# viridityzhu/HiFiHR

Hardware: AMD Instinct MI355X
Metric: train images/sec, FreiHAND 224x224 (ResNet-18 + MANO LBS + render + losses + Adam) (higher is better)
Workload: dtype f32; 1 GPU; BASELINE configs[1]: FreiHAND batch=32/GPU, ResNet-18 encoder + MANO LBS + silhouette/texture render losses, 224x224, aa=3 (672^2 samples); per_gpu_batch=32, global_batch=32, parallelism=dp1

## Files before the change

### hifihr_amd/csrc/conv_halo.hip

```cpp
#include <hip/hip_runtime.h>

#include <cstdlib>
#include <type_traits>

#include "hifihr_internal.h"
#include "lds_dma.h"

namespace hifihr {

namespace {

constexpr int kTW = 14, kTH = 8;
constexpr int kHP = 16;
constexpr int kHaloPix = (kTH + 2) * kHP;
constexpr int kPixF = 68;
constexpr int kHaloPieces = (kHaloPix * kPixF * 4 + 1023) / 1024;
constexpr int kHalo = (kHaloPieces + 1) / 2 * 2 * 256;
constexpr int kWStage = 64 * 64;
constexpr int kStages = 4;
constexpr int kTaps = 9;
constexpr int kNL = 4;
constexpr int kHaloPer = (kHaloPieces + kNL - 1) / kNL;
static_assert(2 * (kTaps - 3) >= kHaloPer, "the next tile's halo is issued two pieces per tap and must land two taps before the tile ends");

// ... 475 lines not shown
      for (int c = 0; c < 4; ++c) R[c] = addsub(raw[c], raw[4 + c], kBneg[i]);
#pragma unroll
      for (int j = 0; j < 4; ++j) {
        V[j] = addsub(R[kBa[j]], R[kBb[j]], kBneg[j]);
        if (HIFIHR_W2_ABLATE == 4) V[j] = raw[j];
      }
    };
    auto fold = [&](int i) {
#pragma unroll
      for (int j = 0; j < 4; ++j)
#pragma unroll
        for (int p = 0; p < 4; ++p) {
          const int co = kAt[p >> 1][i] * kAt[p & 1][j];
          if (co == 1) {
#pragma unroll
            for (int c = 0; c < NCB; ++c) Y[p][c] += M[j][c];
          } else if (co == -1) {
#pragma unroll
            for (int c = 0; c < NCB; ++c) Y[p][c] -= M[j][c];
          }
        }
    };
    read_raw(0);
#if defined(HIFIHR_HALO_STAMP)
    const unsigned long long l0 = HALO_T(), r0 = __builtin_amdgcn_s_memrealtime();
#endif
#pragma unroll
    for (int s = 0; s < kW2Stages; ++s, ++gs) {
#pragma unroll
      for (int q = 0; q < 2; ++q) {
        const int Q = 2 * s + q;
        if (q == 0) {
          read_w(gs, 0, 0);
          if ((s & 1) == 0 && s > 0) fold((s >> 1) - 1);
        }
        transform(Q);
        if (Q + 1 < 2 * kW2Stages) read_raw(Q + 1);
#pragma unroll
        for (int j = 0; j < 4; ++j) {
          if (j < 3) read_w(gs, q, j + 1);
          else if (q == 0) read_w(gs, 1, 0);
#pragma unroll
          for (int k = 0; k < 4; ++k)
#pragma unroll
            for (int c = 0; c < NCB; ++c) {
              const floatx4 acc = ((Q & 3) == 0 && k == 0) ? floatx4{0.f, 0.f, 0.f, 0.f} : M[j][c];
              M[j][c] = __builtin_amdgcn_mfma_f32_16x16x4f32(reinterpret_cast<const float*>(&wv[j & 1][c])[k], comp(V[j], k), acc, 0, 0, 0);
            }
          HIFIHR_SCHED_GROUP(0x100, NCB);
          HIFIHR_SCHED_GROUP(0x008, 4 * NCB);
          HIFIHR_PIN();
        }
      }
#if defined(HIFIHR_HALO_STAMP)
      HIFIHR_TOUCH(M[0][0][0]);
      const unsigned long long b0 = HALO_T();
#endif
      HIFIHR_RAW_BARRIER();
#if defined(HIFIHR_HALO_STAMP)
      st_bar += HALO_T() - b0;
#endif
    }
#if defined(HIFIHR_HALO_STAMP)
    const unsigned long long l1 = HALO_T();
    st_loop += l1 - l0; st_real += __builtin_amdgcn_s_memrealtime() - r0;
#endif
    fold(3);
    if (tt < (t.rows >> 1) * 7 && t.x0 + 2 * (tt % 7) < a.W) {
      const int ty2 = tt / 7, tx2 = tt - 7 * ty2;
#pragma unroll
      for (int c = 0; c < NCB; ++c) {
        const int ch = 16 * (cb0 + c) + 4 * g;
        float4 b4 = make_float4(0.f, 0.f, 0.f, 0.f);
        float4 r4[4] = {b4, b4, b4, b4};
        if constexpr (EPI) {
          if (a.bias != nullptr) b4 = *reinterpret_cast<const float4*>(a.bias + ch);
          if (a.res != nullptr) {
#pragma unroll
            for (int p = 0; p < 4; ++p)
              r4[p] = *reinterpret_cast<const float4*>(a.res + (((size_t)t.n * a.H + t.y0 + 2 * ty2 + (p >> 1)) * a.W + t.x0 + 2 * tx2 + (p & 1)) * 64 + ch);
          }
        }
        auto put = [&](float (&k4)[4], float (&s4)[4], float (&q4)[4], int& n) {
#pragma unroll
          for (int p = 0; p < 4; ++p) {
            float* o = a.dst + (((size_t)t.n * a.H + t.y0 + 2 * ty2 + (p >> 1)) * a.W + t.x0 + 2 * tx2 + (p & 1)) * 64 + ch;
            float4 v = make_float4(Y[p][c][0], Y[p][c][1], Y[p][c][2], Y[p][c][3]);
            if constexpr (EPI) {
              v.x += b4.x + r4[p].x; v.y += b4.y + r4[p].y; v.z += b4.z + r4[p].z; v.w += b4.w + r4[p].w;
              if (a.relu) { v.x = fmaxf(v.x, 0.f); v.y = fmaxf(v.y, 0.f); v.z = fmaxf(v.z, 0.f); v.w = fmaxf(v.w, 0.f); }
            }
            *reinterpret_cast<float4*>(o) = v;
            if constexpr (STATS) {
#if HIFIHR_W2_ABLATE != 7
            if (n == 0) { k4[0] = v.x; k4[1] = v.y; k4[2] = v.z; k4[3] = v.w; }
            const float d0 = v.x - k4[0], d1 = v.y - k4[1], d2 = v.z - k4[2], d3 = v.w - k4[3];
            s4[0] += d0; q4[0] += d0 * d0; s4[1] += d1; q4[1] += d1 * d1;
            s4[2] += d2; q4[2] += d2 * d2; s4[3] += d3; q4[3] += d3 * d3;
            ++n;
#endif
            }
          }
        };
        if (NCB == 2 ? c == 0 : rbw == 0) put(sk[0], ssum[0], ssq[0], sn[0]);
        else put(sk[1], ssum[1], ssq[1], sn[1]);
      }
    }
#if defined(HIFIHR_HALO_STAMP)
    st_epi += HALO_T() - l1;
#endif
  };
  for (int ti = 0; ti < ntiles; ++ti) {
    const Tile t = tile_of(a.H, a.ctiles, cur, s_hi, s_lo, lead);
    cur += t.rows;
    if (t.rows > 4) run_tile(std::integral_constant<int, 2>{}, t, ti & 1);
    else run_tile(std::integral_constant<int, 1>{}, t, ti & 1);
  }
#if defined(HIFIHR_HALO_STAMP)
  if (tid == 0) {
    atomicAdd(&g_halo_stamp[0], st_loop); atomicAdd(&g_halo_stamp[1], st_real); atomicAdd(&g_halo_stamp[2], (unsigned long long)nst);
    atomicAdd(&g_halo_stamp[3], st_bar); atomicAdd(&g_halo_stamp[4], 1ull); atomicAdd(&g_halo_stamp[5], HALO_T() - st_entry);
    atomicAdd(&g_halo_stamp[6], st_epi);
  }
#endif
  if (STATS && a.stats != nullptr) {
#pragma unroll
    for (int s = 0; s < 2; ++s) {
      double S1[4], S2[4];
#pragma unroll
      for (int e = 0; e < 4; ++e) {
        stat_unshift(sn[s], sk[s][e], ssum[s][e], ssq[s][e], S1[e], S2[e]);
        for (int o = 1; o < 16; o <<= 1) { S1[e] += __shfl_xor(S1[e], o, 64); S2[e] += __shfl_xor(S2[e], o, 64); }
      }
      if (r == 0) {
        double* sp = reinterpret_cast<double*>(a.stats) + (size_t)(wg & (stat_slots_used(64) - 1)) * 2 * 64 + 32 * chw + 16 * s + 4 * g;
#pragma unroll
        for (int e = 0; e < 4; ++e) { stat_atomic_add(sp + e, S1[e]); stat_atomic_add(sp + 64 + e, S2[e]); }
      }
    }
  }
}

template <bool EPI, bool STATS>
__global__ __launch_bounds__(256 + 64 * kNL) void conv_wino2_kernel(Wino2Args a) {
  __shared__ __attribute__((aligned(1024))) float lds[2 * kHalo + 2 * kW2Stage];
  wino2_body<EPI, STATS>(a, lds, (int)blockIdx.x, (int)gridDim.x);
}

namespace {
constexpr int kDyT = kTH * kTW * 64;
constexpr int kWgBuf = kHalo + kDyT;
constexpr int kWgPieces = kHaloPieces + kTH * kTW / 4;
constexpr int kWgPer = (kWgPieces + kNL - 1) / kNL;
struct HaloWgradArgs {
  const float* x;
  const float* dy;
  float* slabs;
  const float* zeros;
  int N, H, W;
  int ctiles, total, per;
};
}

__device__ __forceinline__ void halo_wgrad_body(const HaloWgradArgs& a, float* __restrict__ lds, int bid, int nblk) {
  const int tid = threadIdx.x, lane = tid & 63, wave = tid >> 6;
  const int wg = xcd_remap(bid, nblk);
  HaloArgs sh;
  sh.H = a.H; sh.ctiles = a.ctiles;
  const int s_lo = wg * a.per, s_hi = min(s_lo + a.per, a.total);
  int ntiles = 0;
  for (int cur = s_lo; cur < s_hi; cur += tile_at(sh, cur, s_hi).rows) ++ntiles;

  if (wave >= 4) {
    const int l = wave - 4;
    HIFIHR_SET_LOADER_PRIO();
    int pk[kWgPer];
#pragma unroll
    for (int i = 0; i < kWgPer; ++i) {
      const int q = l + kNL * i;
      if (q < kHaloPieces) {
        const int o = q * 1024 + lane * 16;
        const int hp = o / (kPixF * 4), within = o - hp * (kPixF * 4);
        pk[i] = (hp < kHaloPix && within < 256) ? ((hp >> 4) << 12) | ((hp & 15) << 8) | (within >> 4) : -1;
      } else {
        const int p = 4 * (q - kHaloPieces) + (lane >> 4), ty = p / kTW;
        pk[i] = (ty << 16) | ((p - ty * kTW) << 8) | (lane & 15);
      }
    }
    auto issue_tile = [&](const Tile& t, int buf) {
      float* base = lds + buf * kWgBuf;
      const float* ximg = a.x + (size_t)t.n * a.H * a.W * 64;
      const float* dyt = a.dy + (((size_t)t.n * a.H + t.y0) * a.W + t.x0) * 64;
#pragma unroll
      for (int i = 0; i < kWgPer; ++i) {
        const int q = l + kNL * i;
        if (q < kHaloPieces) {
          const int iy = t.y0 - 1 + (pk[i] >> 12), ix = t.x0 - 1 + ((pk[i] >> 8) & 15);
          const bool ok = pk[i] >= 0 && iy >= 0 && iy < a.H && ix >= 0 && ix < a.W;
          HIFIHR_GLDS16(ok ? ximg + (iy * a.W + ix) * 64 + (pk[i] & 15) * 4 : a.zeros, base + 256 * q, lane);
        } else if (q < kWgPieces) {
          const int ty = pk[i] >> 16, tx = (pk[i] >> 8) & 255;
          HIFIHR_GLDS16(ty < t.rows ? dyt + (ty * a.W + tx) * 64 + (pk[i] & 255) * 4 : a.zeros, base + kHalo + 256 * (q - kHaloPieces), lane);
        }
      }
    };
    int cur = s_lo;
    Tile t = tile_at(sh, cur, s_hi);
    if (ntiles > 0) issue_tile(t, 0);
    HIFIHR_WAIT_VM(0);
    HIFIHR_RAW_BARRIER();
    for (int ti = 0; ti < ntiles; ++ti) {
      cur += t.rows;
      if (ti + 1 < ntiles) {
        t = tile_at(sh, cur, s_hi);
        issue_tile(t, (ti + 1) & 1);
      }
      HIFIHR_WAIT_VM(0);
      HIFIHR_RAW_BARRIER();
    }
    return;
  }

  const int r = lane & 15, g = lane >> 4;
  floatx4 acc[kTaps][4];
#pragma unroll
  for (int tp = 0; tp < kTaps; ++tp)
#pragma unroll
    for (int m = 0; m < 4; ++m) acc[tp][m] = floatx4{0.f, 0.f, 0.f, 0.f};
  const char* const lds_b = reinterpret_cast<const char*>(lds);
  const int dy_lane = kHalo * 4 + (4 * r + wave) * 4;
  const int hx_lane = r * 16;

  HIFIHR_RAW_BARRIER();
  int cur = s_lo;
  for (int ti = 0; ti < ntiles; ++ti) {
    const Tile t = tile_at(sh, cur, s_hi);
    cur += t.rows;
    const char* const buf = lds_b + (ti & 1) * (kWgBuf * 4);
    const int ngroups = (t.rows * kTW + 3) >> 2;
    float fy[2];
    float4 fx[2][kTaps];
    auto read_group = [&](int P, int slot) {
      P = min(P, kTH * kTW / 4 - 1);
      const int tpix = 4 * P + g, ty = tpix / kTW;
      const int hpix = ty * kHP + (tpix - ty * kTW);
      fy[slot] = *reinterpret_cast<const float*>(buf + dy_lane + tpix * 256);
      const char* hb = buf + hx_lane + hpix * (kPixF * 4);
#pragma unroll
      for (int tp = 0; tp < kTaps; ++tp) fx[slot][tp] = *reinterpret_cast<const float4*>(hb + ((tp / 3) * kHP + (tp % 3)) * (kPixF * 4));
    };
    auto mfma_group = [&](int slot) {
#pragma unroll
      for (int tp = 0; tp < kTaps; ++tp) {
        acc[tp][0] = __builtin_amdgcn_mfma_f32_16x16x4f32(fy[slot], fx[slot][tp].x, acc[tp][0], 0, 0, 0);
        acc[tp][1] = __builtin_amdgcn_mfma_f32_16x16x4f32(fy[slot], fx[slot][tp].y, acc[tp][1], 0, 0, 0);
        acc[tp][2] = __builtin_amdgcn_mfma_f32_16x16x4f32(fy[slot], fx[slot][tp].z, acc[tp][2], 0, 0, 0);
        acc[tp][3] = __builtin_amdgcn_mfma_f32_16x16x4f32(fy[slot], fx[slot][tp].w, acc[tp][3], 0, 0, 0);
      }
    };
    auto interleave = [&]() {
#pragma unroll
      for (int i = 0; i < kTaps + 1; ++i) {
        HIFIHR_SCHED_GROUP(0x008, 3);
        HIFIHR_SCHED_GROUP(0x100, 1);
        HIFIHR_SCHED_GROUP(0x002, 2);
      }
      HIFIHR_SCHED_GROUP(0x008, 4 * kTaps - 3 * (kTaps + 1));
    };
    read_group(0, 0);
    for (int P = 0; P < ngroups; P += 2) {
      read_group(P + 1, 1);
      mfma_group(0);
      interleave();
      HIFIHR_PIN();
      read_group(P + 2, 0);
      if (P + 1 < ngroups) mfma_group(1);
      interleave();
      HIFIHR_PIN();
    }
    HIFIHR_RAW_BARRIER();
  }
  float* slab = a.slabs + (size_t)wg * (kTaps * 64 * 64);
#pragma unroll
  for (int tp = 0; tp < kTaps; ++tp)
#pragma unroll
    for (int e = 0; e < 4; ++e) {
      const int k = 4 * (4 * g + e) + wave;
      *reinterpret_cast<float4*>(slab + ((size_t)tp * 64 + k) * 64 + 4 * r) = make_float4(acc[tp][0][e], acc[tp][1][e], acc[tp][2][e], acc[tp][3][e]);
    }
}

__global__ __launch_bounds__(256 + 64 * kNL) void conv_halo_wgrad_kernel(HaloWgradArgs a) {
  __shared__ __attribute__((aligned(1024))) float lds[2 * kWgBuf];
  halo_wgrad_body(a, lds, (int)blockIdx.x, (int)gridDim.x);
}

template <bool EPI>
__global__ __launch_bounds__(256 + 64 * kNL) void conv_c64_bwd_pair_kernel(Wino2Args d, int ga, HaloWgradArgs w) {
  constexpr int kPairLds = 2 * kHalo + 2 * kW2Stage > 2 * kWgBuf ? 2 * kHalo + 2 * kW2Stage : 2 * kWgBuf;
  __shared__ __attribute__((aligned(1024))) float lds[kPairLds];
  const int b = (int)blockIdx.x;
  if (b < ga) wino2_body<EPI, false>(d, lds, b, ga);
  else halo_wgrad_body(w, lds, b - ga, (int)gridDim.x - ga);
}

__device__ __forceinline__ void halo_wgrad_reduce_body(const float* __restrict__ slabs, int nslab, float* __restrict__ dw, int blk) {
  __shared__ float part[4][64];
  const int lane = threadIdx.x & 63, w = threadIdx.x >> 6;
  const int i = blk * 64 + lane;
  constexpr size_t kSlab = (size_t)kTaps * 64 * 64;
  float s = 0.f;
  for (int z0 = 16 * w; z0 < nslab; z0 += 64) {
    float v[16];
#pragma unroll
    for (int u = 0; u < 16; ++u) v[u] = (z0 + u < nslab) ? slabs[(size_t)(z0 + u) * kSlab + i] : 0.f;
#pragma unroll
    for (int u = 0; u < 16; ++u) s += v[u];
  }
  part[w][lane] = s;
  __syncthreads();
  if (w == 0) {
    const int c = i & 63, k = (i >> 6) & 63, tp = i >> 12;
    dw[((size_t)k * kTaps + tp) * 64 + c] += (part[0][lane] + part[1][lane]) + (part[2][lane] + part[3][lane]);
  }
}
__global__ __launch_bounds__(256) void conv_halo_wgrad_reduce_kernel(const float* __restrict__ slabs, int nslab, float* __restrict__ dw) {
  halo_wgrad_reduce_body(slabs, nslab, dw, (int)blockIdx.x);
}
constexpr int kHaloReduceMaxJobs = 16;
struct HaloReduceJobs {
  const float* slabs[kHaloReduceMaxJobs];
  float* dw[kHaloReduceMaxJobs];
  int nslab[kHaloReduceMaxJobs];
};
__global__ __launch_bounds__(256) void conv_halo_wgrad_reduce_multi_kernel(HaloReduceJobs js) {
  const int j = blockIdx.y;
  halo_wgrad_reduce_body(js.slabs[j], js.nslab[j], js.dw[j], (int)blockIdx.x);
}

namespace {
constexpr int kSWP = 228;
constexpr int kSHP = 36;
constexpr int kSHRows = 2 * kTH + 5;
constexpr int kSHalo = kSHRows * kSHP * 4;
constexpr int kSPieces = (kSHalo * 4 + 1023) / 1024;
constexpr int kSHaloAl = kSPieces * 256;
struct StemArgs {
  const float* src;
  const float* wgt;
  float* dst;
  float* stats;
  const float* zeros;
  int N, IH, IW, OH, OW;
  int ctiles, total, per;
};
}

__global__ __launch_bounds__(384) void conv_stem_kernel(StemArgs a) {
  __shared__ __attribute__((aligned(1024))) float lds[64 * kSWP + 2 * kSHaloAl];
  float* const wl = lds;
  float* const halo = lds + 64 * kSWP;
  const int tid = threadIdx.x, lane = tid & 63, wave = tid >> 6;
  const int wg = xcd_remap((int)blockIdx.x, (int)gridDim.x);
  HaloArgs sh;
  sh.H = a.OH; sh.ctiles = a.ctiles;
  const int s_lo = wg * a.per, s_hi = min(s_lo + a.per, a.total);
  int ntiles = 0;
  for (int cur = s_lo; cur < s_hi; cur += tile_at(sh, cur, s_hi).rows) ++ntiles;
  __shared__ int c3_any;
  if (tid == 0) c3_any = 0;
  __syncthreads();
  bool c3_mine = false;
  for (int e = tid; e < 64 * 7 * 8; e += 384) {
    const int n = e / 56, rem = e - n * 56, tr = rem >> 3, sl = rem & 7;
    float4 v = make_float4(0.f, 0.f, 0.f, 0.f);
    if (sl < 7) v = *reinterpret_cast<const float4*>(a.wgt + ((size_t)(n * 7 + tr) * 7 + sl) * 4);
    c3_mine = c3_mine || v.w != 0.f;
    *reinterpret_cast<float4*>(wl + n * kSWP + (tr * 8 + sl) * 4) = v;
  }
  if (c3_mine) c3_any = 1;

  if (wave >= 4) {
    HIFIHR_SET_LOADER_PRIO();
    const int l = wave - 4;
    int pk[kSPieces / 2];
#pragma unroll
    for (int i = 0; i < kSPieces / 2; ++i) {
      const int hp = 64 * (l + 2 * i) + lane, hy = hp / kSHP, hx = hp - hy * kSHP;
      pk[i] = (hy < kSHRows && hx < 2 * kTW + 5) ? (hy << 8) | hx : -1;
    }
    auto issue_tile = [&](const Tile& t, int buf) {
      const float* ximg = a.src + (size_t)t.n * a.IH * a.IW * 4;
#pragma unroll
      for (int i = 0; i < kSPieces / 2; ++i) {
        const int iy = 2 * t.y0 - 3 + (pk[i] >> 8), ix = 2 * t.x0 - 3 + (pk[i] & 255);
        const bool ok = pk[i] >= 0 && iy >= 0 && iy < a.IH && ix >= 0 && ix < a.IW;
        HIFIHR_GLDS16(ok ? ximg + (iy * a.IW + ix) * 4 : a.zeros, halo + buf * kSHaloAl + 256 * (l + 2 * i), lane);
      }
    };
    int cur = s_lo;
    Tile t = tile_at(sh, cur, s_hi);
    if (ntiles > 0) issue_tile(t, 0);
    HIFIHR_WAIT_VM(0);
    __syncthreads();
    for (int ti = 0; ti < ntiles; ++ti) {
      cur += t.rows;
      if (ti + 1 < ntiles) {
        t = tile_at(sh, cur, s_hi);
        issue_tile(t, (ti + 1) & 1);
      }
      HIFIHR_WAIT_VM(0);
      HIFIHR_RAW_BARRIER();
    }
    return;
  }

  const int r = lane & 15, g = lane >> 4;
  int hoff[7];
#pragma unroll
  for (int j = 0; j < 7; ++j) {
    const int p = 16 * j + r, ty = p / kTW;
    hoff[j] = ((2 * ty) * kSHP + 2 * (p - ty * kTW) + g) * 16;
  }
  const int woff = (16 * wave + r) * (kSWP * 4) + g * 16;
  const char* const wl_b = reinterpret_cast<const char*>(wl);
  const char* const halo_b = reinterpret_cast<const char*>(halo);
  float ssum[4] = {0.f, 0.f, 0.f, 0.f}, ssq[4] = {0.f, 0.f, 0.f, 0.f}, sk[4] = {0.f, 0.f, 0.f, 0.f};
  int sn = 0;
  __syncthreads();
  const bool c3 = c3_any != 0;
  int cur = s_lo;
  for (int ti = 0; ti < ntiles; ++ti) {
    const Tile t = tile_at(sh, cur, s_hi);
    cur += t.rows;
    const char* const hb = halo_b + (ti & 1) * (kSHaloAl * 4);
    floatx4 acc[7];
#pragma unroll
    for (int j = 0; j < 7; ++j) acc[j] = floatx4{0.f, 0.f, 0.f, 0.f};
    float4 fw[2], fx[2][7];
    auto read_step = [&](int st, int slot) {
      const int tr = st >> 1, kk = st & 1;
      fw[slot] = *reinterpret_cast<const float4*>(wl_b + woff + (tr * 8 + 4 * kk) * 16);
      const char* hs = hb + (tr * kSHP + 4 * kk) * 16;
#pragma unroll
      for (int j = 0; j < 7; ++j) fx[slot][j] = *reinterpret_cast<const float4*>(hs + hoff[j]);
    };
    auto mfma_step = [&](int slot) {
#pragma unroll
      for (int j = 0; j < 7; ++j) acc[j] = __builtin_amdgcn_mfma_f32_16x16x4f32(fw[slot].x, fx[slot][j].x, acc[j], 0, 0, 0);
#pragma unroll
      for (int j = 0; j < 7; ++j) acc[j] = __builtin_amdgcn_mfma_f32_16x16x4f32(fw[slot].y, fx[slot][j].y, acc[j], 0, 0, 0);
#pragma unroll
      for (int j = 0; j < 7; ++j) acc[j] = __builtin_amdgcn_mfma_f32_16x16x4f32(fw[slot].z, fx[slot][j].z, acc[j], 0, 0, 0);
      if (c3) {
#pragma unroll
        for (int j = 0; j < 7; ++j) acc[j] = __builtin_amdgcn_mfma_f32_16x16x4f32(fw[slot].w, fx[slot][j].w, acc[j], 0, 0, 0);
      }
    };
    auto interleave = [&]() {
#pragma unroll
      for (int i = 0; i < 8; ++i) {
        HIFIHR_SCHED_GROUP(0x008, 2);
        HIFIHR_SCHED_GROUP(0x100, 1);
        HIFIHR_SCHED_GROUP(0x002, 1);
      }
      HIFIHR_SCHED_GROUP(0x008, 5);
    };
    read_step(0, 0);
#pragma unroll
    for (int st = 0; st < 14; st += 2) {
      read_step(st + 1, 1);
      mfma_step(0);
      interleave();
      HIFIHR_PIN();
      read_step(st + 2 < 14 ? st + 2 : 13, 0);
      mfma_step(1);
// ... 152 lines not shown
          acc[pr][0] = __builtin_amdgcn_mfma_f32_16x16x4f32(fy[slot], fx[slot][pr].x, acc[pr][0], 0, 0, 0);
          acc[pr][1] = __builtin_amdgcn_mfma_f32_16x16x4f32(fy[slot], fx[slot][pr].y, acc[pr][1], 0, 0, 0);
          acc[pr][2] = __builtin_amdgcn_mfma_f32_16x16x4f32(fy[slot], fx[slot][pr].z, acc[pr][2], 0, 0, 0);
          if (C3) acc[pr][3] = __builtin_amdgcn_mfma_f32_16x16x4f32(fy[slot], fx[slot][pr].w, acc[pr][3], 0, 0, 0);
        }
      };
      auto step = [&](int blk, int q, int rd_slot) {
        read_group(blk, q, rd_slot);
        mfma_group(rd_slot ^ 1);
#pragma unroll
        for (int i = 0; i < 5; ++i) {
          HIFIHR_SCHED_GROUP(0x008, 2);
          HIFIHR_SCHED_GROUP(0x100, 1);
        }
        HIFIHR_SCHED_GROUP(0x008, C3 ? 6 : 2);
        HIFIHR_PIN();
      };
      read_group(0, 0, 0);
      for (int blk = 0; blk < nblk; ++blk) {
        const int nxt = min(blk + 1, kTH / 2 - 1);
        step(blk, 1, 1); step(blk, 2, 0); step(blk, 3, 1); step(blk, 4, 0); step(blk, 5, 1); step(blk, 6, 0); step(nxt, 0, 1);
        if (++blk >= nblk) break;
        const int nx2 = min(blk + 1, kTH / 2 - 1);
        step(blk, 1, 0); step(blk, 2, 1); step(blk, 3, 0); step(blk, 4, 1); step(blk, 5, 0); step(blk, 6, 1); step(nx2, 0, 0);
      }
    };
    if (c3) run_blocks(std::true_type{}); else run_blocks(std::false_type{});
    HIFIHR_RAW_BARRIER();
  }
  float* slab = a.slabs + (size_t)wg * (64 * 196);
  const int trl = r >> 3, sl = r & 7;
#pragma unroll
  for (int pr = 0; pr < 4; ++pr) {
    const int tr = 2 * pr + trl;
    if (tr < 7 && sl < 7) {
#pragma unroll
      for (int e = 0; e < 4; ++e) {
        float* o = slab + (((size_t)(16 * wave + 4 * g + e) * 7 + tr) * 7 + sl) * 4;
        o[0] = acc[pr][0][e]; o[1] = acc[pr][1][e]; o[2] = acc[pr][2][e]; o[3] = acc[pr][3][e];
      }
    }
  }
}

__global__ __launch_bounds__(256) void conv_stem_wgrad_reduce_kernel(const float* __restrict__ slabs, int nslab, float* __restrict__ dw,
                                                                    int dwC) {
  __shared__ float part[4][64];
  const int lane = threadIdx.x & 63, w = threadIdx.x >> 6;
  const int i = blockIdx.x * 64 + lane;
  float s = 0.f;
  for (int z0 = 16 * w; z0 < nslab; z0 += 64) {
    float v[16];
#pragma unroll
    for (int u = 0; u < 16; ++u) v[u] = (z0 + u < nslab) ? slabs[(size_t)(z0 + u) * (64 * 196) + i] : 0.f;
#pragma unroll
    for (int u = 0; u < 16; ++u) s += v[u];
  }
  part[w][lane] = s;
  __syncthreads();
  if (w == 0 && (i & 3) < dwC) dw[(i >> 2) * dwC + (i & 3)] += (part[0][lane] + part[1][lane]) + (part[2][lane] + part[3][lane]);
}

#if defined(HIFIHR_HALO_STAMP)
}
extern "C" int hifihr_halo_stamp_read(unsigned long long* out8, int reset) {
  if (hipMemcpyFromSymbol(out8, HIP_SYMBOL(hifihr::g_halo_stamp), 8 * sizeof(unsigned long long)) != hipSuccess) return 1;
  if (reset) {
    unsigned long long z[8] = {};
    if (hipMemcpyToSymbol(HIP_SYMBOL(hifihr::g_halo_stamp), z, sizeof(z)) != hipSuccess) return 1;
  }
  return 0;
}
namespace hifihr {
#endif

const float* conv_halo_zero_page(hipStream_t st) {
  static float* page[16] = {};
  int dev = 0;
  if (hipGetDevice(&dev) != hipSuccess || dev < 0 || dev >= 16) return nullptr;
  if (page[dev] == nullptr) {
    hipStreamCaptureStatus cs = hipStreamCaptureStatusNone;
    if (hipStreamIsCapturing(st, &cs) != hipSuccess || cs != hipStreamCaptureStatusNone) return nullptr;
    void* p = nullptr;
    if (hipMalloc(&p, 256) != hipSuccess) return nullptr;
    if (hipMemset(p, 0, 256) != hipSuccess) { (void)hipFree(p); return nullptr; }
    page[dev] = static_cast<float*>(p);
  }
  return page[dev];
}

bool conv_halo_supported(const ConvGeom& g, const float* bias) {
  static const int on = [] { const char* e = getenv("HIFIHR_CONV_HALO"); return e ? atoi(e) : 1; }();
  return on && g.R == 3 && g.S == 3 && g.stride == 1 && g.pad == 1 && g.IC == 64 && g.OC == 64 && g.batch <= 1 &&
         !((g.relu || bias != nullptr) && g.dgrad) && g.IH == g.OH && g.IW == g.OW && g.OW >= kTW &&
         (long)g.N * g.OH * g.OW * 64 < (1L << 31);
}

static float* halo_wgrad_scratch(hipStream_t st, size_t bytes) {
  constexpr int kPool = 3;
  struct Dev { bool ready; size_t bytes; float* buf[kPool]; hipStream_t owner[kPool]; int used; };
  static Dev devs[16] = {};
  int dev = 0;
  if (hipGetDevice(&dev) != hipSuccess || dev < 0 || dev >= 16) return nullptr;
  Dev& d = devs[dev];
  if (!d.ready) {
    hipStreamCaptureStatus cs = hipStreamCaptureStatusNone;
    if (hipStreamIsCapturing(st, &cs) != hipSuccess || cs != hipStreamCaptureStatusNone) return nullptr;
    for (int i = 0; i < kPool; ++i) {
      void* p = nullptr;
      if (hipMalloc(&p, bytes) != hipSuccess) return nullptr;
      d.buf[i] = static_cast<float*>(p);
    }
    d.bytes = bytes; d.used = 0; d.ready = true;
  }
  if (bytes > d.bytes) return nullptr;
  for (int i = 0; i < d.used; ++i)
    if (d.owner[i] == st) return d.buf[i];
  if (d.used >= kPool) return nullptr;
  d.owner[d.used] = st;
  return d.buf[d.used++];
}

bool conv_stem_wgrad_supported(const ConvGeom& g) {
  static const int on = [] { const char* e = getenv("HIFIHR_CONV_STEM_WGRAD"); return e ? atoi(e) : 1; }();
  return on && conv_stem_supported(g, nullptr);
}

size_t conv_stem_wgrad_slab_bytes() { return (size_t)device_cus() * 64 * 196 * sizeof(float); }

hipError_t launch_conv_stem_wgrad(const ConvGeom& g, const float* x, const float* dy, float* dw, float* slabs, hipStream_t st, int dw_channels) {
  if (!conv_stem_wgrad_supported(g) || (dw_channels != 3 && dw_channels != 4)) return hipErrorInvalidValue;
  const float* zeros = conv_halo_zero_page(st);
  if (zeros == nullptr) return hipErrorNotReady;
  StemWgradArgs a;
  a.x = x; a.dy = dy; a.zeros = zeros; a.N = g.N; a.IH = g.IH; a.IW = g.IW; a.OH = g.OH; a.OW = g.OW;
  a.ctiles = g.OW / kTW;
  a.total = g.N * a.ctiles * g.OH;
  int G = device_cus();
  a.per = (a.total + G - 1) / G;
  if (a.per < 4) a.per = 4;
  G = (a.total + a.per - 1) / a.per;
  a.slabs = slabs != nullptr ? slabs : halo_wgrad_scratch(st, (size_t)device_cus() * kTaps * 64 * 64 * sizeof(float));
  if (a.slabs == nullptr) return hipErrorNotReady;
  hipLaunchKernelGGL(conv_stem_wgrad_kernel, dim3(G), dim3(512), 0, st, a);
  hipLaunchKernelGGL(conv_stem_wgrad_reduce_kernel, dim3(64 * 196 / 64), dim3(256), 0, st, a.slabs, G, dw, dw_channels);
  return hipGetLastError();
}

bool conv_halo_wgrad_supported(const ConvGeom& g) {
  static const int on = [] { const char* e = getenv("HIFIHR_CONV_HALO_WGRAD"); return e ? atoi(e) : 1; }();
  return on && conv_halo_supported(g, nullptr) && !g.dgrad && g.OW % kTW == 0;
}

size_t conv_halo_wgrad_slab_bytes() { return (size_t)device_cus() * kTaps * 64 * 64 * sizeof(float); }

hipError_t launch_conv_halo_wgrad(const ConvGeom& g, const float* x, const float* dy, float* dw, float* slabs, hipStream_t st) {
  if (!conv_halo_wgrad_supported(g)) return hipErrorInvalidValue;
  const float* zeros = conv_halo_zero_page(st);
  if (zeros == nullptr) return hipErrorNotReady;
  HaloWgradArgs a;
  a.x = x; a.dy = dy; a.zeros = zeros; a.N = g.N; a.H = g.OH; a.W = g.OW;
  a.ctiles = g.OW / kTW;
  a.total = g.N * a.ctiles * g.OH;
  int G = device_cus();
  a.per = (a.total + G - 1) / G;
  if (a.per < 4) a.per = 4;
  G = (a.total + a.per - 1) / a.per;
  a.slabs = slabs != nullptr ? slabs : halo_wgrad_scratch(st, (size_t)device_cus() * kTaps * 64 * 64 * sizeof(float));
  if (a.slabs == nullptr) return hipErrorNotReady;
  hipLaunchKernelGGL(conv_halo_wgrad_kernel, dim3(G), dim3(256 + 64 * kNL), 0, st, a);
  hipLaunchKernelGGL(conv_halo_wgrad_reduce_kernel, dim3(kTaps * 64 * 64 / 64), dim3(256), 0, st, a.slabs, G, dw);
  return hipGetLastError();
}

bool conv_stem_supported(const ConvGeom& g, const float* bias) {
  static const int on = [] { const char* e = getenv("HIFIHR_CONV_STEM"); return e ? atoi(e) : 1; }();
  return on && !g.dgrad && g.R == 7 && g.S == 7 && g.stride == 2 && g.pad == 3 && g.IC == 4 && g.OC == 64 && g.batch <= 1 && !g.relu &&
         bias == nullptr && g.OW % kTW == 0 && (long)g.N * g.OH * g.OW * 64 < (1L << 31);
}

hipError_t launch_conv_stem(const ConvGeom& g, const float* src, const float* wgt, float* dst, float* stats, const float* zeros, hipStream_t st) {
  if (!conv_stem_supported(g, nullptr) || zeros == nullptr) return hipErrorInvalidValue;
  StemArgs a;
  a.src = src; a.wgt = wgt; a.dst = dst; a.stats = stats; a.zeros = zeros;
  a.N = g.N; a.IH = g.IH; a.IW = g.IW; a.OH = g.OH; a.OW = g.OW;
  a.ctiles = g.OW / kTW;
  a.total = g.N * a.ctiles * g.OH;
  int G = device_cus();
  a.per = (a.total + G - 1) / G;
  if (a.per < 4) a.per = 4;
  G = (a.total + a.per - 1) / a.per;
  hipLaunchKernelGGL(conv_stem_kernel, dim3(G), dim3(384), 0, st, a);
  return hipGetLastError();
}

hipError_t launch_conv_halo(const ConvGeom& g, const float* src, const float* wgt, const float* bias, float* dst, float* stats,
                            const float* zeros, hipStream_t st) {
  if (!conv_halo_supported(g, bias) || zeros == nullptr || (stats != nullptr && g.dgrad)) return hipErrorInvalidValue;
  HaloArgs a;
  a.src = src; a.wgt = wgt; a.dst = dst; a.stats = stats; a.zeros = zeros; a.bias = bias; a.relu = g.relu;
  a.N = g.N; a.H = g.OH; a.W = g.OW; a.sign = g.dgrad ? -1 : 1;
  a.ctiles = (g.OW + kTW - 1) / kTW;
  a.total = g.N * a.ctiles * g.OH;
  int G = device_cus();
  a.per = (a.total + G - 1) / G;
  if (a.per < 4) a.per = 4;
  G = (a.total + a.per - 1) / a.per;
  if (bias != nullptr || g.relu || g.OW % kTW != 0) hipLaunchKernelGGL(conv_halo_kernel<true>, dim3(G), dim3(256 + 64 * kNL), 0, st, a);
  else hipLaunchKernelGGL(conv_halo_kernel<false>, dim3(G), dim3(256 + 64 * kNL), 0, st, a);
  return hipGetLastError();
}

bool conv_wino2_supported(int N, int H, int W, int C, int K) {
  static const int on = [] { const char* e = getenv("HIFIHR_CONV_WINO2"); return e ? atoi(e) : 1; }();
  return on && C == 64 && K == 64 && N > 0 && H >= 2 && H % 2 == 0 && W >= kTW && W % 2 == 0 && (long)N * H * W * 64 < (1L << 31);
}

hipError_t launch_conv_wino2(const float* src, const float* U, const float* bias, int relu, float* dst, float* stats, int N, int H, int W,
                             hipStream_t st, const float* res) {
  if (!conv_wino2_supported(N, H, W, 64, 64)) return hipErrorInvalidValue;
  const float* zeros = conv_halo_zero_page(st);
  if (zeros == nullptr) return hipErrorNotReady;
  Wino2Args a;
  a.src = src; a.U = U; a.dst = dst; a.stats = stats; a.zeros = zeros; a.bias = bias; a.relu = relu; a.res = res;
  a.N = N; a.H = H; a.W = W;
  a.ctiles = (W + kTW - 1) / kTW;
  a.total = N * a.ctiles * H;
  int G = device_cus();
  a.per = (a.total + G - 1) / G;
  if (a.per < 4) a.per = 4;
  a.per = (a.per + 1) & ~1;
  G = (a.total + a.per - 1) / a.per;
  if (bias != nullptr || relu || res != nullptr) {
    if (stats != nullptr) hipLaunchKernelGGL((conv_wino2_kernel<true, true>), dim3(G), dim3(256 + 64 * kNL), 0, st, a);
    else hipLaunchKernelGGL((conv_wino2_kernel<true, false>), dim3(G), dim3(256 + 64 * kNL), 0, st, a);
  } else {
    if (stats != nullptr) hipLaunchKernelGGL((conv_wino2_kernel<false, true>), dim3(G), dim3(256 + 64 * kNL), 0, st, a);
    else hipLaunchKernelGGL((conv_wino2_kernel<false, false>), dim3(G), dim3(256 + 64 * kNL), 0, st, a);
  }
  return hipGetLastError();
}

bool conv_c64_bwd_pair_supported(int N, int H, int W) {
  static const int on = [] { const char* e = getenv("HIFIHR_C64_PAIR"); return e ? atoi(e) : 1; }();
  ConvGeom g{};
  g.N = N; g.IH = H; g.IW = W; g.IC = 64; g.OC = 64; g.R = 3; g.S = 3; g.stride = 1; g.pad = 1; g.OH = H; g.OW = W; g.dgrad = 0; g.batch = 1;
  return on && conv_wino2_supported(N, H, W, 64, 64) && conv_halo_wgrad_supported(g) && device_cus() >= 2;
}

hipError_t launch_conv_halo_wgrad_reduce_multi(const HaloReduceJob* jobs, int njobs, hipStream_t st) {
  for (int base = 0; base < njobs; base += kHaloReduceMaxJobs) {
    HaloReduceJobs js;
    const int n = njobs - base < kHaloReduceMaxJobs ? njobs - base : kHaloReduceMaxJobs;
    for (int q = 0; q < n; ++q) {
      if (jobs[base + q].slabs == nullptr || jobs[base + q].dw == nullptr || jobs[base + q].nslab <= 0) return hipErrorInvalidValue;
      js.slabs[q] = jobs[base + q].slabs; js.dw[q] = jobs[base + q].dw; js.nslab[q] = jobs[base + q].nslab;
    }
    hipLaunchKernelGGL(conv_halo_wgrad_reduce_multi_kernel, dim3(kTaps * 64 * 64 / 64, n), dim3(256), 0, st, js);
  }
  return hipGetLastError();
}

hipError_t launch_conv_c64_bwd_pair(const float* dy, const float* U_bwd, const float* res, float* dx, const float* x, float* dw, float* slabs,
                                    int N, int H, int W, hipStream_t st, int* nslab_out) {
  if (!conv_c64_bwd_pair_supported(N, H, W)) return hipErrorInvalidValue;
  const float* zeros = conv_halo_zero_page(st);
  if (zeros == nullptr) return hipErrorNotReady;
  static const int pct = [] { const char* e = getenv("HIFIHR_C64_PAIR_DGRAD_PCT"); int v = e ? atoi(e) : 44; return v < 5 ? 5 : (v > 95 ? 95 : v); }();
  const int cus = device_cus();
  int ga = (cus * pct + 50) / 100;
  if (ga < 1) ga = 1;
  if (ga > cus - 1) ga = cus - 1;
  int gb = cus - ga;
  Wino2Args d;
  d.src = dy; d.U = U_bwd; d.dst = dx; d.stats = nullptr; d.zeros = zeros; d.bias = nullptr; d.relu = 0; d.res = res;
  d.N = N; d.H = H; d.W = W;
  d.ctiles = (W + kTW - 1) / kTW;
  d.total = N * d.ctiles * H;
  d.per = (d.total + ga - 1) / ga;
  if (d.per < 4) d.per = 4;
  d.per = (d.per + 1) & ~1;
  ga = (d.total + d.per - 1) / d.per;
  HaloWgradArgs w;
  w.x = x; w.dy = dy; w.zeros = zeros; w.N = N; w.H = H; w.W = W;
  w.ctiles = W / kTW;
  w.total = N * w.ctiles * H;
  w.per = (w.total + gb - 1) / gb;
  if (w.per < 4) w.per = 4;
  gb = (w.total + w.per - 1) / w.per;
  w.slabs = slabs != nullptr ? slabs : halo_wgrad_scratch(st, (size_t)device_cus() * kTaps * 64 * 64 * sizeof(float));
  if (w.slabs == nullptr) return hipErrorNotReady;
  if (res != nullptr) hipLaunchKernelGGL((conv_c64_bwd_pair_kernel<true>), dim3(ga + gb), dim3(256 + 64 * kNL), 0, st, d, ga, w);
  else hipLaunchKernelGGL((conv_c64_bwd_pair_kernel<false>), dim3(ga + gb), dim3(256 + 64 * kNL), 0, st, d, ga, w);
  if (nslab_out != nullptr) *nslab_out = gb;
  else hipLaunchKernelGGL(conv_halo_wgrad_reduce_kernel, dim3(kTaps * 64 * 64 / 64), dim3(256), 0, st, w.slabs, gb, dw);
  return hipGetLastError();
}

}
```

Baseline: 6672 images/sec.

## Compute 3x3 c64 weight gradient with Winograd F(2x2,3x3) split across workgroup pairs

Replaces the direct 9-tap MFMA weight-gradient accumulation with a Winograd-domain formulation. Input and dy tiles are transformed and accumulated into 16 transform-domain products, split into two halves of 8 handled by paired workgroups. The reduce kernel sums the half-slabs and applies the output transform back to 3x3 taps. This aims to cut MFMA work per tile, in exchange for extra transform ALU work, a restructured job/slab partitioning, and a changed reduce layout with possible numerical differences.

```diff
diff --git a/hifihr_amd/csrc/conv_halo.hip b/hifihr_amd/csrc/conv_halo.hip
--- a/hifihr_amd/csrc/conv_halo.hip
+++ b/hifihr_amd/csrc/conv_halo.hip
@@ -651,24 +651,126 @@
 constexpr int kWgBuf = kHalo + kDyT;
 constexpr int kWgPieces = kHaloPieces + kTH * kTW / 4;
 constexpr int kWgPer = (kWgPieces + kNL - 1) / kNL;
+constexpr int kWgSteps = (kTH / 2) * (kTW / 2) / 4;
+constexpr int kWgSlab = 8 * 64 * 64;
+static_assert(2 * kWgSlab <= 2 * kTaps * 64 * 64, "two position-half slabs per pair of workgroups fit the documented workspace (9 x 64 x 64 floats per CU)");
 struct HaloWgradArgs {
   const float* x;
   const float* dy;
   float* slabs;
   const float* zeros;
   int N, H, W;
-  int ctiles, total, per;
+  int ctiles, total, per, shares;
 };
+
+constexpr int wg_tile_offs(int T) {
+  const int tr = T / (kTW / 2), ix = T - tr * (kTW / 2), tc = 2 * ix < kTW / 2 ? 2 * ix : 2 * ix - kTW / 2;
+  return ((2 * tr * kTW + 2 * tc) * 256) | (((2 * tr * kHP + 2 * tc) * (kPixF * 4)) << 16);
+}
+static_assert((kTH * kTW) * 256 < (1 << 16) && kHaloPix * kPixF * 4 < (1 << 16), "the packed offsets are 16 bits each");
+__device__ __forceinline__ float f4c(const float4& v, int m) { return m == 0 ? v.x : m == 1 ? v.y : m == 2 ? v.z : v.w; }
+
+template <int HALF>
+__device__ __forceinline__ void wino_wgrad_mfma(const float* __restrict__ lds, int ntiles, int lane, int wave, float* __restrict__ slab) {
+  const int r = lane & 15, g = lane >> 4;
+  floatx4 acc[8][4];
+#pragma unroll
+  for (int p = 0; p < 8; ++p)
+#pragma unroll
+    for (int m = 0; m < 4; ++m) acc[p][m] = floatx4{0.f, 0.f, 0.f, 0.f};
+  const int dy_lane = kHalo * 4 + r * 16, hx_lane = HALF * kHP * (kPixF * 4) + (16 * wave + r) * 4;
+  const char* const lds_b = reinterpret_cast<const char*>(lds);
+  float4 fd[2][2][2];
+  float fx[3][4];
+  float v[2][2][4];
+  auto read_step = [&](const char* buf, int P, int slot) {
+    int gg = g;
+    HIFIHR_TOUCH(gg);
+    const int o = gg == 0 ? wg_tile_offs(4 * P) : gg == 1 ? wg_tile_offs(4 * P + 1) : gg == 2 ? wg_tile_offs(4 * P + 2) : wg_tile_offs(4 * P + 3);
+    const char* db = buf + dy_lane + (o & 0xffff);
+    const char* hb = buf + hx_lane + ((unsigned)o >> 16);
+#pragma unroll
+    for (int j = 0; j < 3; ++j)
+#pragma unroll
+      for (int q = 0; q < 4; ++q) fx[j][q] = *reinterpret_cast<const float*>(hb + (j * kHP + q) * (kPixF * 4));
+#pragma unroll
+    for (int a = 0; a < 2; ++a)
+#pragma unroll
+      for (int b = 0; b < 2; ++b) fd[slot][a][b] = *reinterpret_cast<const float4*>(db + (a * kTW + b) * 256);
+  };
+  auto x_transform = [&](int slot) {
+#pragma unroll
+    for (int i = 0; i < 2; ++i) {
+      float t[4];
+#pragma unroll
+      for (int q = 0; q < 4; ++q) {
+        if (HALF == 0) t[q] = i == 0 ? fx[0][q] - fx[2][q] : fx[1][q] + fx[2][q];
+        else t[q] = i == 0 ? fx[1][q] - fx[0][q] : fx[0][q] - fx[2][q];
+      }
+      v[slot][i][0] = t[0] - t[2]; v[slot][i][1] = t[1] + t[2]; v[slot][i][2] = t[2] - t[1]; v[slot][i][3] = t[1] - t[3];
+    }
+  };
+  auto mfma_block = [&](int slot, int m) {
+    const float d00 = f4c(fd[slot][0][0], m), d01 = f4c(fd[slot][0][1], m), d10 = f4c(fd[slot][1][0], m), d11 = f4c(fd[slot][1][1], m);
+    float u[2][2];
+    if (HALF == 0) { u[0][0] = d00; u[0][1] = d01; u[1][0] = d00 + d10; u[1][1] = d01 + d11; }
+    else { u[0][0] = d00 - d10; u[0][1] = d01 - d11; u[1][0] = d10; u[1][1] = d11; }
+#pragma unroll
+    for (int i = 0; i < 2; ++i) {
+      const float w1 = u[i][0] + u[i][1], w2 = u[i][0] - u[i][1];
+      acc[4 * i + 0][m] = __builtin_amdgcn_mfma_f32_16x16x4f32(u[i][0], v[slot][i][0], acc[4 * i + 0][m], 0, 0, 0);
+      acc[4 * i + 1][m] = __builtin_amdgcn_mfma_f32_16x16x4f32(w1, v[slot][i][1], acc[4 * i + 1][m], 0, 0, 0);
+      acc[4 * i + 2][m] = __builtin_amdgcn_mfma_f32_16x16x4f32(w2, v[slot][i][2], acc[4 * i + 2][m], 0, 0, 0);
+      acc[4 * i + 3][m] = __builtin_amdgcn_mfma_f32_16x16x4f32(u[i][1], v[slot][i][3], acc[4 * i + 3][m], 0, 0, 0);
+    }
+  };
+  auto step = [&](int slot, const char* next_buf, int next_P) {
+    read_step(next_buf, next_P, slot ^ 1);
+    mfma_block(slot, 0);
+    HIFIHR_PIN();
+    mfma_block(slot, 1);
+    HIFIHR_PIN();
+    mfma_block(slot, 2);
+    HIFIHR_PIN();
+    mfma_block(slot, 3);
+    x_transform(slot ^ 1);
+    HIFIHR_PIN();
+  };
+  auto tile = [&](auto par, int ti) {
+    constexpr int S = decltype(par)::value;
+    const char* const buf = lds_b + (ti & 1) * (kWgBuf * 4);
+#pragma unroll
+    for (int P = 0; P < kWgSteps - 1; ++P) step((P + S) & 1, buf, P + 1);
+    HIFIHR_WAIT_LGKM0();
+    HIFIHR_RAW_BARRIER();
+    step((kWgSteps - 1 + S) & 1, lds_b + ((ti + 1) & 1) * (kWgBuf * 4), 0);
+  };
+
+  HIFIHR_RAW_BARRIER();
+  if (ntiles > 0) { read_step(lds_b, 0, 0); x_transform(0); }
+  HIFIHR_PIN();
+  for (int ti = 0; ti < ntiles; ti += 2) {
+    tile(std::integral_constant<int, 0>{}, ti);
+    if (ti + 1 < ntiles) tile(std::integral_constant<int, 1>{}, ti + 1);
+  }
+#pragma unroll
+  for (int p = 0; p < 8; ++p)
+#pragma unroll
+    for (int e = 0; e < 4; ++e)
+      *reinterpret_cast<float4*>(slab + ((size_t)p * 64 + 16 * wave + r) * 64 + 4 * (4 * g + e)) = make_float4(acc[p][0][e], acc[p][1][e], acc[p][2][e], acc[p][3][e]);
+}
 }
 
 __device__ __forceinline__ void halo_wgrad_body(const HaloWgradArgs& a, float* __restrict__ lds, int bid, int nblk) {
   const int tid = threadIdx.x, lane = tid & 63, wave = tid >> 6;
-  const int wg = xcd_remap(bid, nblk);
   HaloArgs sh;
   sh.H = a.H; sh.ctiles = a.ctiles;
-  const int s_lo = wg * a.per, s_hi = min(s_lo + a.per, a.total);
-  int ntiles = 0;
-  for (int cur = s_lo; cur < s_hi; cur += tile_at(sh, cur, s_hi).rows) ++ntiles;
+  const int job0 = xcd_remap(bid, nblk);
+  auto count_tiles = [&](int s_lo, int s_hi) {
+    int n = 0;
+    for (int cur = s_lo; cur < s_hi; cur += tile_at(sh, cur, s_hi).rows) ++n;
+    return n;
+  };
 
   if (wave >= 4) {
     const int l = wave - 4;
@@ -703,90 +805,34 @@
         }
       }
     };
-    int cur = s_lo;
-    Tile t = tile_at(sh, cur, s_hi);
-    if (ntiles > 0) issue_tile(t, 0);
-    HIFIHR_WAIT_VM(0);
-    HIFIHR_RAW_BARRIER();
-    for (int ti = 0; ti < ntiles; ++ti) {
-      cur += t.rows;
-      if (ti + 1 < ntiles) {
-        t = tile_at(sh, cur, s_hi);
-        issue_tile(t, (ti + 1) & 1);
-      }
+    for (int job = job0; job < 2 * a.shares; job += nblk) {
+      const int s_lo = (job >> 1) * a.per, s_hi = min(s_lo + a.per, a.total);
+      const int ntiles = count_tiles(s_lo, s_hi);
+      int cur = s_lo;
+      Tile t = tile_at(sh, cur, s_hi);
+      if (ntiles > 0) issue_tile(t, 0);
       HIFIHR_WAIT_VM(0);
       HIFIHR_RAW_BARRIER();
+      for (int ti = 0; ti < ntiles; ++ti) {
+        cur += t.rows;
+        if (ti + 1 < ntiles) {
+          t = tile_at(sh, cur, s_hi);
+          issue_tile(t, (ti + 1) & 1);
+        }
+        HIFIHR_WAIT_VM(0);
+        HIFIHR_RAW_BARRIER();
+      }
     }
     return;
   }
 
-  const int r = lane & 15, g = lane >> 4;
-  floatx4 acc[kTaps][4];
-#pragma unroll
-  for (int tp = 0; tp < kTaps; ++tp)
-#pragma unroll
-    for (int m = 0; m < 4; ++m) acc[tp][m] = floatx4{0.f, 0.f, 0.f, 0.f};
-  const char* const lds_b = reinterpret_cast<const char*>(lds);
-  const int dy_lane = kHalo * 4 + (4 * r + wave) * 4;
-  const int hx_lane = r * 16;
-
-  HIFIHR_RAW_BARRIER();
-  int cur = s_lo;
-  for (int ti = 0; ti < ntiles; ++ti) {
-    const Tile t = tile_at(sh, cur, s_hi);
-    cur += t.rows;
-    const char* const buf = lds_b + (ti & 1) * (kWgBuf * 4);
-    const int ngroups = (t.rows * kTW + 3) >> 2;
-    float fy[2];
-    float4 fx[2][kTaps];
-    auto read_group = [&](int P, int slot) {
-      P = min(P, kTH * kTW / 4 - 1);
-      const int tpix = 4 * P + g, ty = tpix / kTW;
-      const int hpix = ty * kHP + (tpix - ty * kTW);
-      fy[slot] = *reinterpret_cast<const float*>(buf + dy_lane + tpix * 256);
-      const char* hb = buf + hx_lane + hpix * (kPixF * 4);
-#pragma unroll
-      for (int tp = 0; tp < kTaps; ++tp) fx[slot][tp] = *reinterpret_cast<const float4*>(hb + ((tp / 3) * kHP + (tp % 3)) * (kPixF * 4));
-    };
-    auto mfma_group = [&](int slot) {
-#pragma unroll
-      for (int tp = 0; tp < kTaps; ++tp) {
-        acc[tp][0] = __builtin_amdgcn_mfma_f32_16x16x4f32(fy[slot], fx[slot][tp].x, acc[tp][0], 0, 0, 0);
-        acc[tp][1] = __builtin_amdgcn_mfma_f32_16x16x4f32(fy[slot], fx[slot][tp].y, acc[tp][1], 0, 0, 0);
-        acc[tp][2] = __builtin_amdgcn_mfma_f32_16x16x4f32(fy[slot], fx[slot][tp].z, acc[tp][2], 0, 0, 0);
-        acc[tp][3] = __builtin_amdgcn_mfma_f32_16x16x4f32(fy[slot], fx[slot][tp].w, acc[tp][3], 0, 0, 0);
-      }
-    };
-    auto interleave = [&]() {
-#pragma unroll
-      for (int i = 0; i < kTaps + 1; ++i) {
-        HIFIHR_SCHED_GROUP(0x008, 3);
-        HIFIHR_SCHED_GROUP(0x100, 1);
-        HIFIHR_SCHED_GROUP(0x002, 2);
-      }
-      HIFIHR_SCHED_GROUP(0x008, 4 * kTaps - 3 * (kTaps + 1));
-    };
-    read_group(0, 0);
-    for (int P = 0; P < ngroups; P += 2) {
-      read_group(P + 1, 1);
-      mfma_group(0);
-      interleave();
-      HIFIHR_PIN();
-      read_group(P + 2, 0);
-      if (P + 1 < ngroups) mfma_group(1);
-      interleave();
-      HIFIHR_PIN();
-    }
-    HIFIHR_RAW_BARRIER();
-  }
-  float* slab = a.slabs + (size_t)wg * (kTaps * 64 * 64);
-#pragma unroll
-  for (int tp = 0; tp < kTaps; ++tp)
-#pragma unroll
-    for (int e = 0; e < 4; ++e) {
-      const int k = 4 * (4 * g + e) + wave;
-      *reinterpret_cast<float4*>(slab + ((size_t)tp * 64 + k) * 64 + 4 * r) = make_float4(acc[tp][0][e], acc[tp][1][e], acc[tp][2][e], acc[tp][3][e]);
-    }
+  for (int job = job0; job < 2 * a.shares; job += nblk) {
+    const int s_lo = (job >> 1) * a.per, s_hi = min(s_lo + a.per, a.total);
+    const int ntiles = count_tiles(s_lo, s_hi);
+    float* slab = a.slabs + (size_t)job * kWgSlab;
+    if (job & 1) wino_wgrad_mfma<1>(lds, ntiles, lane, wave, slab);
+    else wino_wgrad_mfma<0>(lds, ntiles, lane, wave, slab);
+  }
 }
 
 __global__ __launch_bounds__(256 + 64 * kNL) void conv_halo_wgrad_kernel(HaloWgradArgs a) {
@@ -803,24 +849,54 @@
   else halo_wgrad_body(w, lds, b - ga, (int)gridDim.x - ga);
 }
 
+constexpr int kWgRedElems = 32;
 __device__ __forceinline__ void halo_wgrad_reduce_body(const float* __restrict__ slabs, int nslab, float* __restrict__ dw, int blk) {
-  __shared__ float part[4][64];
-  const int lane = threadIdx.x & 63, w = threadIdx.x >> 6;
-  const int i = blk * 64 + lane;
-  constexpr size_t kSlab = (size_t)kTaps * 64 * 64;
-  float s = 0.f;
-  for (int z0 = 16 * w; z0 < nslab; z0 += 64) {
-    float v[16];
-#pragma unroll
-    for (int u = 0; u < 16; ++u) v[u] = (z0 + u < nslab) ? slabs[(size_t)(z0 + u) * kSlab + i] : 0.f;
-#pragma unroll
-    for (int u = 0; u < 16; ++u) s += v[u];
-  }
-  part[w][lane] = s;
+  __shared__ float part[8][8][kWgRedElems];
+  const int l = threadIdx.x & 31, sub = threadIdx.x >> 5, h = sub & 1, q = sub >> 1;
+  const int i = blk * kWgRedElems + l;
+  const int nshare = nslab >> 1;
+  float s[8];
+#pragma unroll
+  for (int p = 0; p < 8; ++p) s[p] = 0.f;
+  for (int z = q; z < nshare; z += 8) {
+    float v[2][8];
+#pragma unroll
+    for (int u = 0; u < 2; ++u)
+#pragma unroll
+      for (int p = 0; p < 8; ++p) v[u][p] = (z + 4 * u < nshare) ? slabs[((size_t)(2 * (z + 4 * u) + h) * 8 + p) * 4096 + i] : 0.f;
+#pragma unroll
+    for (int u = 0; u < 2; ++u)
+#pragma unroll
+      for (int p = 0; p < 8; ++p) s[p] += v[u][p];
+  }
+#pragma unroll
+  for (int p = 0; p < 8; ++p) part[sub][p][l] = s[p];
   __syncthreads();
-  if (w == 0) {
-    const int c = i & 63, k = (i >> 6) & 63, tp = i >> 12;
-    dw[((size_t)k * kTaps + tp) * 64 + c] += (part[0][lane] + part[1][lane]) + (part[2][lane] + part[3][lane]);
+  if (sub == 0) {
+    float U[4][4];
+#pragma unroll
+    for (int pi = 0; pi < 4; ++pi)
+#pragma unroll
+      for (int pj = 0; pj < 4; ++pj) {
+        const int hh = pi >> 1, p = 4 * (pi & 1) + pj;
+        const float t = (part[hh][p][l] + part[2 + hh][p][l]) + (part[4 + hh][p][l] + part[6 + hh][p][l]);
+        U[pi][pj] = ((pi == 3) != (pj == 3)) ? -t : t;
+      }
+    float R[3][4];
+#pragma unroll
+    for (int pj = 0; pj < 4; ++pj) {
+      const float a = 0.5f * (U[1][pj] + U[2][pj]), b = 0.5f * (U[1][pj] - U[2][pj]);
+      R[0][pj] = U[0][pj] + a; R[1][pj] = b; R[2][pj] = a + U[3][pj];
+    }
+    const int c = i >> 6, k = i & 63;
+    float* o = dw + (size_t)k * kTaps * 64 + c;
+#pragma unroll
+    for (int ta = 0; ta < 3; ++ta) {
+      const float a = 0.5f * (R[ta][1] + R[ta][2]), b = 0.5f * (R[ta][1] - R[ta][2]);
+      o[(ta * 3 + 0) * 64] += R[ta][0] + a;
+      o[(ta * 3 + 1) * 64] += b;
+      o[(ta * 3 + 2) * 64] += a + R[ta][3];
+    }
   }
 }
 __global__ __launch_bounds__(256) void conv_halo_wgrad_reduce_kernel(const float* __restrict__ slabs, int nslab, float* __restrict__ dw) {
@@ -1279,6 +1355,21 @@
   return on && conv_halo_supported(g, nullptr) && !g.dgrad && g.OW % kTW == 0;
 }
 
+static int halo_wgrad_workgroups(int avail) {
+  const char* e = getenv("HIFIHR_HALO_WGRAD_WGS");
+  const int v = e ? atoi(e) : 0;
+  return v > 0 && v < avail ? v : avail;
+}
+
+static int halo_wgrad_split(HaloWgradArgs& a, int wgs) {
+  int shares = wgs >= 2 ? wgs / 2 : 1;
+  a.per = (a.total + shares - 1) / shares;
+  if (a.per < 4) a.per = 4;
+  a.shares = (a.total + a.per - 1) / a.per;
+  if ((size_t)2 * a.shares * kWgSlab > (size_t)device_cus() * kTaps * 64 * 64) return 0;
+  return wgs >= 2 ? 2 * a.shares : 1;
+}
+
 size_t conv_halo_wgrad_slab_bytes() { return (size_t)device_cus() * kTaps * 64 * 64 * sizeof(float); }
 
 hipError_t launch_conv_halo_wgrad(const ConvGeom& g, const float* x, const float* dy, float* dw, float* slabs, hipStream_t st) {
@@ -1289,14 +1380,12 @@
   a.x = x; a.dy = dy; a.zeros = zeros; a.N = g.N; a.H = g.OH; a.W = g.OW;
   a.ctiles = g.OW / kTW;
   a.total = g.N * a.ctiles * g.OH;
-  int G = device_cus();
-  a.per = (a.total + G - 1) / G;
-  if (a.per < 4) a.per = 4;
-  G = (a.total + a.per - 1) / a.per;
+  const int G = halo_wgrad_split(a, halo_wgrad_workgroups(device_cus()));
+  if (G == 0) return hipErrorInvalidValue;
   a.slabs = slabs != nullptr ? slabs : halo_wgrad_scratch(st, (size_t)device_cus() * kTaps * 64 * 64 * sizeof(float));
   if (a.slabs == nullptr) return hipErrorNotReady;
   hipLaunchKernelGGL(conv_halo_wgrad_kernel, dim3(G), dim3(256 + 64 * kNL), 0, st, a);
-  hipLaunchKernelGGL(conv_halo_wgrad_reduce_kernel, dim3(kTaps * 64 * 64 / 64), dim3(256), 0, st, a.slabs, G, dw);
+  hipLaunchKernelGGL(conv_halo_wgrad_reduce_kernel, dim3(64 * 64 / kWgRedElems), dim3(256), 0, st, a.slabs, 2 * a.shares, dw);
   return hipGetLastError();
 }
 
@@ -1383,7 +1472,7 @@
       if (jobs[base + q].slabs == nullptr || jobs[base + q].dw == nullptr || jobs[base + q].nslab <= 0) return hipErrorInvalidValue;
       js.slabs[q] = jobs[base + q].slabs; js.dw[q] = jobs[base + q].dw; js.nslab[q] = jobs[base + q].nslab;
     }
-    hipLaunchKernelGGL(conv_halo_wgrad_reduce_multi_kernel, dim3(kTaps * 64 * 64 / 64, n), dim3(256), 0, st, js);
+    hipLaunchKernelGGL(conv_halo_wgrad_reduce_multi_kernel, dim3(64 * 64 / kWgRedElems, n), dim3(256), 0, st, js);
   }
   return hipGetLastError();
 }
@@ -1398,6 +1487,7 @@
   int ga = (cus * pct + 50) / 100;
   if (ga < 1) ga = 1;
   if (ga > cus - 1) ga = cus - 1;
+  if (((cus - ga) & 1) && cus - ga > 1) ++ga;
   int gb = cus - ga;
   Wino2Args d;
   d.src = dy; d.U = U_bwd; d.dst = dx; d.stats = nullptr; d.zeros = zeros; d.bias = nullptr; d.relu = 0; d.res = res;
@@ -1412,15 +1502,14 @@
   w.x = x; w.dy = dy; w.zeros = zeros; w.N = N; w.H = H; w.W = W;
   w.ctiles = W / kTW;
   w.total = N * w.ctiles * H;
-  w.per = (w.total + gb - 1) / gb;
-  if (w.per < 4) w.per = 4;
-  gb = (w.total + w.per - 1) / w.per;
+  gb = halo_wgrad_split(w, halo_wgrad_workgroups(gb));
+  if (gb == 0) return hipErrorInvalidValue;
   w.slabs = slabs != nullptr ? slabs : halo_wgrad_scratch(st, (size_t)device_cus() * kTaps * 64 * 64 * sizeof(float));
   if (w.slabs == nullptr) return hipErrorNotReady;
   if (res != nullptr) hipLaunchKernelGGL((conv_c64_bwd_pair_kernel<true>), dim3(ga + gb), dim3(256 + 64 * kNL), 0, st, d, ga, w);
   else hipLaunchKernelGGL((conv_c64_bwd_pair_kernel<false>), dim3(ga + gb), dim3(256 + 64 * kNL), 0, st, d, ga, w);
-  if (nslab_out != nullptr) *nslab_out = gb;
-  else hipLaunchKernelGGL(conv_halo_wgrad_reduce_kernel, dim3(kTaps * 64 * 64 / 64), dim3(256), 0, st, w.slabs, gb, dw);
+  if (nslab_out != nullptr) *nslab_out = 2 * w.shares;
+  else hipLaunchKernelGGL(conv_halo_wgrad_reduce_kernel, dim3(64 * 64 / kWgRedElems), dim3(256), 0, st, w.slabs, 2 * w.shares, dw);
   return hipGetLastError();
 }
 
```

Result: no change. 6732 images/sec, median of 6 (+0.9%).
